# eladhoffer/convNet.pytorch

Measured on NVIDIA H100. Metric: ResNet-50 images/sec (training step, synthetic 224x224), higher is better.
Workload: dtype bf16

## Files before the change

### convnet/pytorch_b200/csrc/conv3x3.cu

```cuda
#include "common.cuh"
#include "host.h"
#include <stdlib.h>

namespace b200 {

constexpr int kHThreads = 384;
constexpr int kHTileM = 128;
constexpr int kHMaxA = 6, kHMaxB = 8;
constexpr int kHMaxTaps = 16;
constexpr int kHStatReplicas = 16;

struct HaloParams {
  int N, H, W, C, Kout;
  int RT, Wp;
  int tiles_per_img, m_tiles, n_tiles, block_n, c_chunks;
  int sa, sb;
  uint32_t a_bytes, a_box_bytes, b_bytes;
  int act;
  int has_res;
  double* stats;
  const float* bias;
  int ntaps, pad;
  int row_bytes;
  int b_stationary;
  int diag;
  uint16_t a_off[kHMaxTaps];
  uint16_t b_tap[kHMaxTaps];
};

template <int NTAPS, int KSTEPS, int BN>
__global__ void __launch_bounds__(kHThreads, 1)
conv_halo_kernel(const __grid_constant__ CUtensorMap tmX, const __grid_constant__ CUtensorMap tmB,
                 const __grid_constant__ CUtensorMap tmC, const __grid_constant__ CUtensorMap tmR,
                 const __grid_constant__ HaloParams p) {
  extern __shared__ uint8_t smem_raw[];
  __shared__ __align__(8) uint64_t a_full[kHMaxA], a_empty[kHMaxA], b_full[kHMaxB], b_empty[kHMaxB];
  __shared__ __align__(8) uint64_t res_bar, bstat_bar;

  const int warp = threadIdx.x >> 5, lane = threadIdx.x & 31;
  const uint32_t raw_addr = smem_u32(smem_raw);
  uint8_t* smem = smem_raw + (((raw_addr + 1023u) & ~1023u) - raw_addr);
  uint8_t* sA = smem;
  uint8_t* sB = sA + p.sa * p.a_bytes;
  const int b_slots = p.b_stationary ? p.c_chunks * p.ntaps : p.sb;
  uint8_t* epi = sB + b_slots * p.b_bytes;

  if (threadIdx.x == 0) {
    for (int i = 0; i < p.sa; ++i) { mbar_init(&a_full[i], 1); mbar_init(&a_empty[i], 8); }
    for (int i = 0; i < kHMaxB; ++i) { mbar_init(&b_full[i], 1); mbar_init(&b_empty[i], 8); }
    mbar_init(&bstat_bar, 1);
    mbar_init(&res_bar, 1);
    fence_mbar_init();
    prefetch_tmap(&tmX); prefetch_tmap(&tmB); prefetch_tmap(&tmC);
    if (p.has_res) prefetch_tmap(&tmR);
  }
  __syncthreads();
  pdl_wait();
  const int t_start = p.diag ? static_cast<int>(blockIdx.x) / p.n_tiles : static_cast<int>(blockIdx.x);
  const int t_step = p.diag ? static_cast<int>(gridDim.x) / p.n_tiles : static_cast<int>(gridDim.x);
  const int total_tiles = p.diag ? p.m_tiles : p.m_tiles * p.n_tiles;
  const int own_n = static_cast<int>(blockIdx.x) % p.n_tiles;

  if (warp >= 8) {
    producer_setmaxnreg();
    if (warp == 8 && lane == 0) {
      int ia = 0, ib = 0; uint32_t pa = 0, pb = 0;
      const int cw = p.row_bytes >> 1;
      if (p.b_stationary && t_start < total_tiles) {
        mbar_arrive_expect_tx(&bstat_bar, static_cast<uint32_t>(p.c_chunks * NTAPS) * p.b_bytes);
        for (int cc = 0; cc < p.c_chunks; ++cc)
          for (int t = 0; t < NTAPS; ++t)
            tma_load_3d(&tmB, &bstat_bar, sB + (cc * NTAPS + t) * p.b_bytes, cc * cw, p.b_tap[t],
                        p.diag ? own_n * p.block_n : 0);
      }
      for (int tile = t_start; tile < total_tiles; tile += t_step) {
        const int m_tile = p.diag ? tile : tile / p.n_tiles, n_tile = p.diag ? own_n : tile - m_tile * p.n_tiles;
        const int img = m_tile / p.tiles_per_img;
        const int h0 = (m_tile - img * p.tiles_per_img) * p.RT;
        for (int cc = 0; cc < p.c_chunks; ++cc) {
          mbar_wait(&a_empty[ia], pa ^ 1u);
          mbar_arrive_expect_tx(&a_full[ia], p.a_box_bytes);
          tma_load_4d(&tmX, &a_full[ia], sA + ia * p.a_bytes, (p.diag ? n_tile : cc) * cw, -p.pad, h0 - p.pad, img);
          if (++ia == p.sa) { ia = 0; pa ^= 1u; }
          if (p.b_stationary) continue;
          for (int t = 0; t < NTAPS; ++t) {
            mbar_wait(&b_empty[ib], pb ^ 1u);
            mbar_arrive_expect_tx(&b_full[ib], p.b_bytes);
            tma_load_3d(&tmB, &b_full[ib], sB + ib * p.b_bytes, cc * cw, p.b_tap[t], n_tile * p.block_n);
            if (++ib == p.sb) { ib = 0; pb ^= 1u; }
          }
        }
      }
    }
    return;
  }
  consumer_setmaxnreg();

  const int wg = warp >> 2;
  const int r_lo = wg * 64 + (warp & 3) * 16 + (lane >> 2);
  const int c_lo = 2 * (lane & 3);
  const bool leader = threadIdx.x == 0;
  const uint64_t proto = make_smem_desc(0, 16, 8u * p.row_bytes, layout_type_for_row_bytes(p.row_bytes));
  const uint32_t a_wg = (64u * wg * p.row_bytes) >> 4;
  const int nbox = BN >> 6;
  const uint32_t box_bytes = static_cast<uint32_t>(p.RT * p.W) * 128u;
  const uint32_t box_pitch = (box_bytes + 1023u) & ~1023u;
  int srow[2];
  bool in_tile[2];
#pragma unroll
  for (int h = 0; h < 2; ++h) {
    const int v = r_lo + 8 * h;
    const int ry = v / p.Wp, cx = v - ry * p.Wp;
    srow[h] = ry * p.W + cx;
    in_tile[h] = (ry < p.RT) && (cx < p.W);
  }
  const int st_col = threadIdx.x % BN;
  const int st_rows = kHTileM / (256 / BN);
  const int st_row0 = (threadIdx.x / BN) * st_rows;
  int st_ntile = -1;
  float st_s1 = 0.f, st_s2 = 0.f;
  if (p.b_stationary && t_start < total_tiles) mbar_wait(&bstat_bar, 0);

  float acc[BN / 2];
  int ia = 0, ib = 0; uint32_t pa = 0, pb = 0;
  int local = 0;
  for (int tile = t_start; tile < total_tiles; tile += t_step, ++local) {
    const int m_tile = p.diag ? tile : tile / p.n_tiles, n_tile = p.diag ? own_n : tile - m_tile * p.n_tiles;
    const int img = m_tile / p.tiles_per_img;
    const int h0 = (m_tile - img * p.tiles_per_img) * p.RT;
    const int nbase = n_tile * BN;
    if (leader && local > 0) bulk_wait_group_read0();
    named_bar_sync(1, 256);
    if (leader && p.has_res) {
      fence_proxy_async();
      mbar_arrive_expect_tx(&res_bar, static_cast<uint32_t>(nbox) * box_bytes);
      for (int b = 0; b < nbox; ++b) tma_load_4d(&tmR, &res_bar, epi + b * box_pitch, nbase + b * 64, 0, h0, img);
    }

    wgmma_fence_acc(acc);
    int rel_a = -1, rel_b = -1;
    for (int cc = 0; cc < p.c_chunks; ++cc) {
      mbar_wait(&a_full[ia], pa);
      const uint64_t da0 = proto + (smem_u32(sA + ia * p.a_bytes) >> 4) + a_wg;
#pragma unroll
      for (int t = 0; t < NTAPS; ++t) {
        uint64_t db0;
        if (p.b_stationary) {
          db0 = proto + (smem_u32(sB + (cc * NTAPS + t) * p.b_bytes) >> 4);
        } else {
          mbar_wait(&b_full[ib], pb);
          db0 = proto + (smem_u32(sB + ib * p.b_bytes) >> 4);
        }
        const uint32_t tap_inc = (static_cast<uint32_t>(p.a_off[t]) * p.row_bytes) >> 4;
        wgmma_fence();
#pragma unroll
        for (int k = 0; k < KSTEPS; ++k)
          wgmma_bf16<0, 0>(acc, da0 + tap_inc + 2 * k, db0 + 2 * k, (cc | t | k) != 0 ? 1u : 0u);
        if (!p.b_stationary || t == NTAPS - 1) {
          wgmma_commit();
          wgmma_wait<1>();
          if (rel_b >= 0) release_stage(&b_empty[rel_b], lane);
          if (rel_a >= 0) release_stage(&a_empty[rel_a], lane);
          rel_a = (t == NTAPS - 1) ? ia : -1;
          rel_b = p.b_stationary ? -1 : ib;
        }
        if (!p.b_stationary && ++ib == p.sb) { ib = 0; pb ^= 1u; }
      }
      if (++ia == p.sa) { ia = 0; pa ^= 1u; }
    }
    wgmma_wait<0>();
    wgmma_fence_acc(acc);
    if (rel_b >= 0) release_stage(&b_empty[rel_b], lane);
    if (rel_a >= 0) release_stage(&a_empty[rel_a], lane);

    if (p.has_res) mbar_wait(&res_bar, static_cast<uint32_t>(local & 1));
#pragma unroll
    for (int h = 0; h < 2; ++h) {
      if (!in_tile[h] || h0 + (r_lo + 8 * h) / p.Wp >= p.H) continue;
      const int row = srow[h];
#pragma unroll
      for (int j = 0; j < BN / 2; j += 4) {
        const int c = 2 * j + c_lo;
        {
          uint32_t* dst = reinterpret_cast<uint32_t*>(epi + (c >> 6) * box_pitch + row * 128 +
                                                      ((((c & 63) >> 3) ^ (row & 7)) << 4) + (c & 7) * 2);
          float v0 = acc[j + 2 * h], v1 = acc[j + 2 * h + 1];
          if (p.bias != nullptr) { v0 += __ldg(p.bias + nbase + c); v1 += __ldg(p.bias + nbase + c + 1); }
          if (p.has_res) {
            const float2 t2 = unpack_bf16x2(*dst);
            v0 += t2.x;
            v1 += t2.y;
          }
          *dst = pack_bf16x2(apply_act(v0, p.act), apply_act(v1, p.act));
        }
      }
    }
    fence_proxy_async();
    named_bar_sync(1, 256);
    if (leader) {
      for (int b = 0; b < nbox; ++b) tma_store_4d(&tmC, epi + b * box_pitch, nbase + b * 64, 0, h0, img);
      bulk_commit_group();
    }
    if (p.stats != nullptr) {
      if (st_ntile != n_tile) {
        if (st_ntile >= 0) {
          double* dst = p.stats + (blockIdx.x % kHStatReplicas) * 2 * p.Kout + st_ntile * BN + st_col;
          atomicAdd(dst, (double)st_s1);
          atomicAdd(dst + p.Kout, (double)st_s2);
        }
        st_ntile = n_tile; st_s1 = 0.f; st_s2 = 0.f;
      }
      const int vrows = min(p.RT, p.H - h0) * p.W;
      const uint8_t* col = epi + (st_col >> 6) * box_pitch + (st_col & 7) * 2;
      const int j = (st_col & 63) >> 3;
      const int r_end = min(st_row0 + st_rows, vrows);
      for (int r = st_row0; r < r_end; ++r) {
        const float x = __bfloat162float(*reinterpret_cast<const __nv_bfloat16*>(col + r * 128 + ((j ^ (r & 7)) << 4)));
        st_s1 += x;
        st_s2 = fmaf(x, x, st_s2);
      }
    }
  }
  if (p.stats != nullptr && st_ntile >= 0) {
    double* dst = p.stats + (blockIdx.x % kHStatReplicas) * 2 * p.Kout + st_ntile * BN + st_col;
    atomicAdd(dst, (double)st_s1);
    atomicAdd(dst + p.Kout, (double)st_s2);
  }
  if (leader) bulk_wait_group0();
}

typedef void (*HaloKernelFn)(const __grid_constant__ CUtensorMap, const __grid_constant__ CUtensorMap,
                             const __grid_constant__ CUtensorMap, const __grid_constant__ CUtensorMap,
                             const __grid_constant__ HaloParams);
static HaloKernelFn halo_kernel_for(int ntaps, int block_n) {
  if (ntaps == 9)
    return block_n == 64 ? conv_halo_kernel<9, 4, 64> : block_n == 128 ? conv_halo_kernel<9, 4, 128>
         : block_n == 256 ? conv_halo_kernel<9, 4, 256> : nullptr;
  if (ntaps == 16)
    return block_n == 64 ? conv_halo_kernel<16, 1, 64> : block_n == 128 ? conv_halo_kernel<16, 1, 128>
         : block_n == 256 ? conv_halo_kernel<16, 1, 256> : nullptr;
  return nullptr;
}

static int enc4(CUtensorMap* tm, const void* base, int C, int W, int H, int N, int b0, int b1, int b2) {
  EncodeTiledFn fn = encode_tiled_fn();
  B200_REQUIRE(fn != nullptr, B200_ERR_CUDA, "cuTensorMapEncodeTiled entry point unavailable");
  cuuint64_t dims[4] = {(cuuint64_t)C, (cuuint64_t)W, (cuuint64_t)H, (cuuint64_t)N};
  cuuint64_t strides[3] = {(cuuint64_t)C * 2, (cuuint64_t)W * C * 2, (cuuint64_t)H * W * C * 2};
  cuuint32_t box[4] = {(cuuint32_t)b0, (cuuint32_t)b1, (cuuint32_t)b2, 1};
  cuuint32_t es[4] = {1, 1, 1, 1};
  CUresult r = fn(tm, CU_TENSOR_MAP_DATA_TYPE_BFLOAT16, 4, const_cast<void*>(base), dims, strides, box, es,
                  CU_TENSOR_MAP_INTERLEAVE_NONE, swizzle_for_row_bytes(b0 * 2), CU_TENSOR_MAP_L2_PROMOTION_L2_128B,
                  CU_TENSOR_MAP_FLOAT_OOB_FILL_NONE);
  B200_REQUIRE(r == CUDA_SUCCESS, B200_ERR_CUDA, "cuTensorMapEncodeTiled(4d) failed (%d) dims=(%d,%d,%d,%d) box=(%d,%d,%d)",
               (int)r, C, W, H, N, b0, b1, b2);
  return B200_OK;
}

static bool halo_enabled() {
  static const bool enabled = !(getenv("B200_HALO") && atoi(getenv("B200_HALO")) == 0);
  return enabled;
}

bool halo_geometry_ok(int H, int W, int Cs, int R, int S, int pad) {
  if (!halo_enabled()) return false;
  const bool k3 = (R == 3 && S == 3 && pad == 1 && Cs % 64 == 0);
  const bool k4 = (R == 4 && S == 4 && pad == 0 && Cs == 16);
  if (!k3 && !k4) return false;
  const int Wp = W + S - 1;
  if (Wp > 128 || W < 8) return false;
  int RT = 128 / Wp;
  if (RT > H) RT = H;
  const int tiles = (H + RT - 1) / RT;
  return (double)H * W / (128.0 * tiles) >= 0.6;
}

bool halo_eligible(int H, int W, int Cs, int Nout, int R, int S, int pad) {
  if (!halo_geometry_ok(H, W, Cs, R, S, pad) || Nout % 64 != 0) return false;
  const int n_tiles = (Nout + 255) / 256;
  const int block_n = Nout / n_tiles;
  return Nout % n_tiles == 0 && block_n % 64 == 0 && 256 % block_n == 0;
}

int launch_halo(const void* src, const void* wmat, void* out, const void* res, const float* bias, int N, int H, int W,
                int Cs, int Nout, int R, int S, int pad, int dir, int act, double* stats, cudaStream_t stream, int window) {
  HaloParams p;
  memset(&p, 0, sizeof(p));
  p.diag = window > 0 ? 1 : 0;
  if (p.diag)
    B200_REQUIRE(window == 64 && Cs == Nout && Cs % 64 == 0 && R == 3 && S == 3, B200_ERR_UNSUPPORTED,
                 "conv halo: window mode needs window == 64, C == K, C %% 64 == 0 and a 3x3 filter (C=%d K=%d)", Cs, Nout);
  p.N = N; p.H = H; p.W = W; p.C = Cs; p.Kout = Nout;
  p.ntaps = R * S; p.pad = pad;
  p.row_bytes = (Cs == 16) ? 32 : 128;
  const int cw = p.row_bytes / 2;
  p.Wp = W + S - 1;
  p.RT = 128 / p.Wp;
  if (p.RT > H) p.RT = H;
  p.tiles_per_img = (H + p.RT - 1) / p.RT;
  p.m_tiles = N * p.tiles_per_img;
  p.n_tiles = p.diag ? Nout / 64 : (Nout + 255) / 256;
  p.block_n = Nout / p.n_tiles;
  p.c_chunks = p.diag ? 1 : Cs / cw;
  p.a_box_bytes = (uint32_t)(p.RT + R - 1) * p.Wp * p.row_bytes;
  uint32_t a_need = (uint32_t)(kHTileM + (R - 1) * p.Wp + (S - 1)) * p.row_bytes;
  if (a_need < p.a_box_bytes) a_need = p.a_box_bytes;
  p.a_bytes = (a_need + 1023u) & ~1023u;
  p.b_bytes = (uint32_t)p.block_n * p.row_bytes;
  p.act = act;
  p.has_res = res != nullptr;
  p.stats = stats;
  p.bias = bias;
  for (int r = 0; r < R; ++r)
    for (int s = 0; s < S; ++s) {
      const int t = r * S + s;
      p.b_tap[t] = (uint16_t)t;
      p.a_off[t] = (uint16_t)(dir == 0 ? r * p.Wp + s : (R - 1 - r) * p.Wp + (S - 1 - s));
    }
  const uint32_t box_pitch = (((uint32_t)(p.RT * W) * 128u) + 1023u) & ~1023u;
  const uint32_t epi_bytes = (uint32_t)(p.block_n / 64) * box_pitch;
  int budget = 212 * 1024 - (int)epi_bytes;
  const int b_all = p.c_chunks * p.ntaps * (int)p.b_bytes;
  p.b_stationary = ((p.n_tiles == 1 || p.diag) && b_all <= 80 * 1024) ? 1 : 0;
  B200_REQUIRE(!p.diag || p.b_stationary, B200_ERR_UNSUPPORTED, "conv halo: window mode expects resident weights");
  int b_region;
  if (p.b_stationary) {
    b_region = b_all;
    p.sb = 0;
    p.sa = (budget - b_region) / (int)p.a_bytes;
    if (p.sa > kHMaxA) p.sa = kHMaxA;
  } else {
    p.sa = 2;
    p.sb = (budget - p.sa * (int)p.a_bytes) / (int)p.b_bytes;
    if (p.sb > kHMaxB) p.sb = kHMaxB;
    if (p.sb >= 6 && (int)(3 * p.a_bytes + 4 * p.b_bytes) <= budget) {
      p.sa = 3;
      p.sb = (budget - 3 * (int)p.a_bytes) / (int)p.b_bytes;
      if (p.sb > kHMaxB) p.sb = kHMaxB;
    }
    b_region = p.sb * (int)p.b_bytes;
  }
  B200_REQUIRE(p.sa >= 2 && (p.b_stationary || p.sb >= 2), B200_ERR_UNSUPPORTED,
               "conv halo: shared memory budget exceeded (W=%d, block_n=%d)", W, p.block_n);
  CUtensorMap tmX, tmB, tmC, tmR;
  memset(&tmR, 0, sizeof(tmR));
  int rc = enc4(&tmX, src, Cs, W + S - 1 - 2 * pad, H + R - 1 - 2 * pad, N, cw, p.Wp, p.RT + R - 1);
  if (rc) return rc;
  {
    EncodeTiledFn fn = encode_tiled_fn();
    const int wc = p.diag ? window : Cs;
    cuuint64_t dims[3] = {(cuuint64_t)wc, (cuuint64_t)p.ntaps, (cuuint64_t)Nout};
    cuuint64_t strides[2] = {(cuuint64_t)wc * 2, (cuuint64_t)wc * p.ntaps * 2};
    cuuint32_t box[3] = {(cuuint32_t)cw, 1, (cuuint32_t)p.block_n};
    cuuint32_t es[3] = {1, 1, 1};
    CUresult r = fn(&tmB, CU_TENSOR_MAP_DATA_TYPE_BFLOAT16, 3, const_cast<void*>(wmat), dims, strides, box, es,
                    CU_TENSOR_MAP_INTERLEAVE_NONE, swizzle_for_row_bytes(p.row_bytes),
                    CU_TENSOR_MAP_L2_PROMOTION_L2_128B, CU_TENSOR_MAP_FLOAT_OOB_FILL_NONE);
    B200_REQUIRE(r == CUDA_SUCCESS, B200_ERR_CUDA, "conv halo: weight tensor map failed (%d)", (int)r);
  }
  rc = enc4(&tmC, out, Nout, W, H, N, 64, W, p.RT);
  if (rc) return rc;
  if (res) {
    rc = enc4(&tmR, res, Nout, W, H, N, 64, W, p.RT);
    if (rc) return rc;
  }
  const int smem_bytes = p.sa * (int)p.a_bytes + b_region + (int)epi_bytes + 1024;
  HaloKernelFn kfn = halo_kernel_for(p.ntaps, p.block_n);
  B200_REQUIRE(kfn != nullptr, B200_ERR_UNSUPPORTED, "conv halo: %d taps with block_n %d unsupported", p.ntaps, p.block_n);
  cudaError_t e = cudaFuncSetAttribute((const void*)kfn, cudaFuncAttributeMaxDynamicSharedMemorySize, smem_bytes);
  B200_REQUIRE(e == cudaSuccess, B200_ERR_CUDA, "conv halo: smem attribute (%d bytes): %s", smem_bytes, cudaGetErrorString(e));
  const int total = p.m_tiles * p.n_tiles;
  int grid = total < sm_count() ? total : sm_count();
  if (p.diag) {
    int per_n = sm_count() / p.n_tiles;
    if (per_n > p.m_tiles) per_n = p.m_tiles;
    if (per_n < 1) per_n = 1;
    grid = per_n * p.n_tiles;
  }
  if (getenv("B200_HALO_DEBUG"))
    fprintf(stderr, "[halo] dir=%d N=%d H=%d W=%d C=%d K=%d taps=%d block_n=%d n_tiles=%d m_tiles=%d bstat=%d diag=%d "
            "sa=%d sb=%d bias=%d res=%d act=%d stats=%d grid=%d\n", dir, N, H, W, Cs, Nout, p.ntaps, p.block_n,
            p.n_tiles, p.m_tiles, p.b_stationary, p.diag, p.sa, p.sb, bias != nullptr, res != nullptr, act,
            stats != nullptr, grid);
  b200::launch(kfn, grid, kHThreads, smem_bytes, stream, tmX, tmB, tmC, tmR, p);
  B200_CHECK_LAUNCH("conv_halo_kernel");
  return B200_OK;
}


constexpr int kWThreads = 384;
constexpr int kWMaxStages = 4;

struct HaloWgradParams {
  int N, H, W, K_out, C;
  int RT, Wp, tiles_per_img, m_tiles;
  int ntaps, pad, halo_rows;
  int x_row_bytes, cw, ncols;
  int c_chunks, k_tiles, units, splits, tiles_per_split;
  int stages;
  int window;
  uint32_t a_box_bytes, a_bytes, x_box_bytes, x_bytes;
  float* partial;
  uint16_t x_off[kHMaxTaps];
};

template <int R, int S>
__global__ void __launch_bounds__(kWThreads, 1)
conv_halo_wgrad_kernel(const __grid_constant__ CUtensorMap tmDy, const __grid_constant__ CUtensorMap tmX,
                       const __grid_constant__ HaloWgradParams p) {
  constexpr int kCols = S * 16;
  extern __shared__ uint8_t smem_raw[];
  __shared__ __align__(8) uint64_t full_bar[kWMaxStages], empty_bar[kWMaxStages];
  const int warp = threadIdx.x >> 5, lane = threadIdx.x & 31;
  const uint32_t raw_addr = smem_u32(smem_raw);
  uint8_t* smem = smem_raw + (((raw_addr + 1023u) & ~1023u) - raw_addr);
  const uint32_t stage_bytes = p.a_bytes + p.x_bytes;

  {
    uint4* z = reinterpret_cast<uint4*>(smem);
    const int n16 = static_cast<int>(p.stages * stage_bytes) >> 4;
    for (int i = threadIdx.x; i < n16; i += kWThreads) z[i] = make_uint4(0u, 0u, 0u, 0u);
  }
  if (threadIdx.x == 0) {
    for (int s = 0; s < p.stages; ++s) { mbar_init(&full_bar[s], 1); mbar_init(&empty_bar[s], 8); }
    fence_mbar_init();
    prefetch_tmap(&tmDy);
    prefetch_tmap(&tmX);
  }
  fence_proxy_async();
  __syncthreads();
  pdl_wait();

  const int split = blockIdx.x / p.units;
  const int unit = blockIdx.x - split * p.units;
  const int k_tile = unit % p.k_tiles;
  const int cc = unit / p.k_tiles;
  const int k0 = k_tile * kHTileM;
  const int t_begin = split * p.tiles_per_split;
  const int t_end = min(p.m_tiles, t_begin + p.tiles_per_split);
  const int ntiles = t_end - t_begin;
  const int nA = min(2, (p.K_out - k0 + 63) / 64);
  if (ntiles <= 0) return;

  if (warp >= 8) {
    producer_setmaxnreg();
    if (warp == 8 && lane == 0) {
      int stage = 0; uint32_t phase = 0;
      const uint32_t tx = nA * p.a_box_bytes + p.x_box_bytes;
      for (int tile = t_begin; tile < t_end; ++tile) {
        const int img = tile / p.tiles_per_img;
        const int h0 = (tile - img * p.tiles_per_img) * p.RT;
        mbar_wait(&empty_bar[stage], phase ^ 1u);
        uint8_t* sa = smem + stage * stage_bytes;
        mbar_arrive_expect_tx(&full_bar[stage], tx);
        for (int j = 0; j < nA; ++j) tma_load_4d(&tmDy, &full_bar[stage], sa + j * 16384, k0 + j * 64, 0, h0, img);
        tma_load_4d(&tmX, &full_bar[stage], sa + p.a_bytes, cc * p.cw + (p.window ? k0 : 0), -p.pad, h0 - p.pad, img);
        if (++stage == p.stages) { stage = 0; phase ^= 1u; }
      }
    }
    return;
  }
  consumer_setmaxnreg();

  const int wg = warp >> 2;
  const bool wg_on = wg < nA;
  const uint64_t protoA = make_smem_desc(0, 16384, 1024, 1);
  const uint64_t protoX = make_smem_desc(0, p.x_row_bytes, 8u * p.x_row_bytes, layout_type_for_row_bytes(p.x_row_bytes));
  uint32_t row_inc[R];
#pragma unroll
  for (int r = 0; r < R; ++r) row_inc[r] = (static_cast<uint32_t>(p.x_off[r * S]) * p.x_row_bytes) >> 4;
  const uint32_t kx_inc = (16u * p.x_row_bytes) >> 4;
  float acc[R][kCols / 2];
#pragma unroll
  for (int r = 0; r < R; ++r) wgmma_fence_acc(acc[r]);
  int stage = 0, prev = 0; uint32_t phase = 0;
  for (int i = 0; i < ntiles; ++i) {
    mbar_wait(&full_bar[stage], phase);
    if (wg_on) {
      const uint32_t a_addr = smem_u32(smem + stage * stage_bytes);
      const uint64_t da0 = protoA + ((a_addr + wg * 16384) >> 4);
      const uint64_t dx0 = protoX + ((a_addr + p.a_bytes) >> 4);
      wgmma_fence();
#pragma unroll
      for (int k = 0; k < 8; ++k) {
        const uint32_t scale = (k != 0 || i != 0) ? 1u : 0u;
#pragma unroll
        for (int r = 0; r < R; ++r)
          wgmma_bf16<1, 1>(acc[r], da0 + k * 128, dx0 + row_inc[r] + k * kx_inc, scale);
      }
      wgmma_commit();
      wgmma_wait<1>();
    }
    if (i > 0) release_stage(&empty_bar[prev], lane);
    prev = stage;
    if (++stage == p.stages) { stage = 0; phase ^= 1u; }
  }
  wgmma_wait<0>();
#pragma unroll
  for (int r = 0; r < R; ++r) wgmma_fence_acc(acc[r]);
  release_stage(&empty_bar[prev], lane);
  if (!wg_on) return;

  const int row = wg * 64 + (warp & 3) * 16 + (lane >> 2);
  const int c_lo = 2 * (lane & 3);
#pragma unroll
  for (int h = 0; h < 2; ++h) {
    float* dst = p.partial + ((static_cast<long long>(unit) * p.splits + split) * kHTileM + row + 8 * h) * p.ncols;
#pragma unroll
    for (int r = 0; r < R; ++r)
#pragma unroll
      for (int j = 0; j < kCols / 2; j += 4)
        *reinterpret_cast<float2*>(dst + r * kCols + 2 * j + c_lo) = make_float2(acc[r][j + 2 * h], acc[r][j + 2 * h + 1]);
  }
}

__global__ void __launch_bounds__(256) conv_halo_wgrad_reduce_kernel(const float* __restrict__ partial,
                                                                     float* __restrict__ dw, int K_out, int ntaps, int C,
                                                                     int cw, int k_tiles, int splits, int ncols) {
  pdl_wait();
  __shared__ float4 red[8][32];
  const int c4n = C >> 2;
  const long long total = static_cast<long long>(K_out) * ntaps * c4n;
  const int lane = threadIdx.x & 31, w = threadIdx.x >> 5, nw = blockDim.x >> 5;
  for (long long base = static_cast<long long>(blockIdx.x) * 32; base < total; base += static_cast<long long>(gridDim.x) * 32) {
    const long long idx = base + lane;
    float4 acc = make_float4(0.f, 0.f, 0.f, 0.f);
    int c = 0, tap = 0, k = 0;
    if (idx < total) {
      c = static_cast<int>(idx % c4n) * 4;
      tap = static_cast<int>((idx / c4n) % ntaps);
      k = static_cast<int>(idx / (static_cast<long long>(c4n) * ntaps));
      const int k_tile = k >> 7, row = k & 127;
      const int cc = c / cw;
      const int unit = cc * k_tiles + k_tile;
      const float* src = partial + ((static_cast<long long>(unit) * splits) * kHTileM + row) * ncols + tap * cw + (c - cc * cw);
      for (int s2 = w; s2 < splits; s2 += nw) {
        const float4 v = __ldcg(reinterpret_cast<const float4*>(src + static_cast<long long>(s2) * kHTileM * ncols));
        acc.x += v.x; acc.y += v.y; acc.z += v.z; acc.w += v.w;
      }
    }
    red[w][lane] = acc;
    __syncthreads();
    if (w == 0 && idx < total) {
      for (int j = 1; j < nw; ++j) {
        const float4 v = red[j][lane];
        acc.x += v.x; acc.y += v.y; acc.z += v.z; acc.w += v.w;
      }
      float4* d = reinterpret_cast<float4*>(dw + (static_cast<long long>(k) * ntaps + tap) * C + c);
      float4 o = *d;
      o.x += acc.x; o.y += acc.y; o.z += acc.z; o.w += acc.w;
      *d = o;
    }
    __syncthreads();
  }
}

bool halo_wgrad_eligible(int H, int W, int C, int K_out, int R, int S, int pad) {
  static const bool enabled = !(getenv("B200_HALO_WGRAD") && atoi(getenv("B200_HALO_WGRAD")) == 0);
  if (!enabled || !halo_geometry_ok(H, W, C, R, S, pad)) return false;
  return K_out % 64 == 0;
}

int launch_halo_wgrad(const void* x, const void* dy, float* dw, void* workspace, size_t workspace_bytes, int N, int H,
                      int W, int C, int K_out, int R, int S, int pad, cudaStream_t stream, int window) {
  HaloWgradParams p;
  memset(&p, 0, sizeof(p));
  p.window = window;
  if (window)
    B200_REQUIRE(window == 128 && C == K_out && C % 128 == 0, B200_ERR_UNSUPPORTED,
                 "conv halo wgrad: window mode needs window == 128 and C == K, C %% 128 == 0 (C=%d K=%d)", C, K_out);
  p.N = N; p.H = H; p.W = W; p.K_out = K_out; p.C = C;
  p.ntaps = R * S; p.pad = pad;
  p.cw = 16;
  p.x_row_bytes = p.cw * 2;
  p.ncols = p.ntaps * p.cw;
  p.Wp = W + S - 1;
  p.RT = 128 / p.Wp;
  if (p.RT > H) p.RT = H;
  p.halo_rows = p.RT + R - 1;
  p.tiles_per_img = (H + p.RT - 1) / p.RT;
  p.m_tiles = N * p.tiles_per_img;
  p.c_chunks = (window ? window : C) / p.cw;
  p.k_tiles = (K_out + kHTileM - 1) / kHTileM;
  p.units = p.c_chunks * p.k_tiles;
  int splits = sm_count() / p.units;
  if (splits < 1) splits = 1;
  if (splits > p.m_tiles) splits = p.m_tiles;
  p.tiles_per_split = (p.m_tiles + splits - 1) / splits;
  p.splits = (p.m_tiles + p.tiles_per_split - 1) / p.tiles_per_split;
  p.a_box_bytes = (uint32_t)(p.RT * p.Wp) * 128u;
  p.a_bytes = 2 * 16384;
  p.x_box_bytes = (uint32_t)(p.halo_rows * p.Wp) * p.x_row_bytes;
  int max_off = 0;
  for (int r = 0; r < R; ++r)
    for (int s = 0; s < S; ++s) {
      p.x_off[r * S + s] = (uint16_t)(r * p.Wp + s);
      if (r * p.Wp + s > max_off) max_off = r * p.Wp + s;
    }
  uint32_t x_need = (uint32_t)(kHTileM + max_off) * p.x_row_bytes;
  if (x_need < p.x_box_bytes) x_need = p.x_box_bytes;
  p.x_bytes = (x_need + 1023u) & ~1023u;
  p.stages = (212 * 1024) / (int)(p.a_bytes + p.x_bytes);
  if (p.stages > kWMaxStages) p.stages = kWMaxStages;
  B200_REQUIRE(p.stages >= 2, B200_ERR_UNSUPPORTED, "conv halo wgrad: shared memory budget exceeded (W=%d)", W);
  const size_t need = (size_t)p.units * p.splits * kHTileM * p.ncols * sizeof(float);
  B200_REQUIRE(workspace != nullptr && workspace_bytes >= need, B200_ERR_INVALID,
               "conv halo wgrad: workspace of %zu bytes needed (%zu given)", need, workspace_bytes);
  p.partial = reinterpret_cast<float*>(workspace);
  CUtensorMap tmDy, tmX;
  int rc = enc4(&tmDy, dy, K_out, W, H, N, 64, p.Wp, p.RT);
  if (rc) return rc;
  rc = enc4(&tmX, x, C, W + S - 1 - 2 * pad, H + R - 1 - 2 * pad, N, p.cw, p.Wp, p.halo_rows);
  if (rc) return rc;
  const int smem_bytes = p.stages * (int)(p.a_bytes + p.x_bytes) + 1024;
  const void* kfn = (p.ntaps == 9) ? (const void*)conv_halo_wgrad_kernel<3, 3> : (const void*)conv_halo_wgrad_kernel<4, 4>;
  cudaError_t e = cudaFuncSetAttribute(kfn, cudaFuncAttributeMaxDynamicSharedMemorySize, smem_bytes);
  B200_REQUIRE(e == cudaSuccess, B200_ERR_CUDA, "conv halo wgrad: smem attribute (%d bytes): %s", smem_bytes,
               cudaGetErrorString(e));
  if (getenv("B200_HALO_DEBUG"))
    fprintf(stderr, "[halo_wgrad] N=%d H=%d W=%d C=%d K=%d taps=%d k_tiles=%d c_chunks=%d m_tiles=%d units=%d "
            "splits=%d tiles_per_split=%d stages=%d grid=%d\n", N, H, W, C, K_out, p.ntaps, p.k_tiles, p.c_chunks,
            p.m_tiles, p.units, p.splits, p.tiles_per_split, p.stages, p.units * p.splits);
  if (p.ntaps == 9)
    b200::launch(conv_halo_wgrad_kernel<3, 3>, p.units * p.splits, kWThreads, smem_bytes, stream, tmDy, tmX, p);
  else
    b200::launch(conv_halo_wgrad_kernel<4, 4>, p.units * p.splits, kWThreads, smem_bytes, stream, tmDy, tmX, p);
  B200_CHECK_LAUNCH("conv_halo_wgrad_kernel");
  const int Cw = window ? window : C;
  const long long total = (long long)K_out * p.ntaps * (Cw / 4);
  long long blocks64 = (total + 31) / 32;
  if (blocks64 > 16LL * sm_count()) blocks64 = 16LL * sm_count();
  const int blocks = (int)blocks64;
  b200::launch(conv_halo_wgrad_reduce_kernel, blocks, 32 * wgrad_reduce_warps(p.splits), 0, stream, p.partial, dw, K_out, p.ntaps, Cw, p.cw, p.k_tiles, p.splits,
                                                            p.ncols);
  B200_CHECK_LAUNCH("conv_halo_wgrad_reduce_kernel");
  return B200_OK;
}

}
```

Before: 5474.

## Alternate consumer warpgroups over 128-row tiles so epilogue overlaps MMA

Before, both consumer warpgroups each took 64 rows of one tile. Now each warpgroup computes a full 128-row tile (two M-halves of wgmma) on its own, and the two groups alternate tile-halves. A turn barrier hands the mainloop from one group to the other, so one group's epilogue (bias, residual, activation, TMA store, BN statistics) can overlap the other's MMAs. Wide block_n is split into 128-column passes, which reloads the A tile for each pass. The epilogue buffer doubles to one per warpgroup, which takes shared memory away from the pipeline stages. Weights can no longer stay resident when block_n is split.

```diff
diff --git a/convnet/pytorch_b200/csrc/conv3x3.cu b/convnet/pytorch_b200/csrc/conv3x3.cu
--- a/convnet/pytorch_b200/csrc/conv3x3.cu
+++ b/convnet/pytorch_b200/csrc/conv3x3.cu
@@ -28,14 +28,25 @@
   uint16_t b_tap[kHMaxTaps];
 };
 
-template <int NTAPS, int KSTEPS, int BN>
+template <int KSTEPS, int SZ>
+__device__ __forceinline__ void halo_tap_mma(float (&acc)[2][SZ], uint64_t da, uint64_t db, uint32_t a_half,
+                                             uint32_t scale0) {
+  wgmma_fence();
+#pragma unroll
+  for (int k = 0; k < KSTEPS; ++k) {
+    wgmma_bf16<0, 0>(acc[0], da + 2 * k, db + 2 * k, k != 0 ? 1u : scale0);
+    wgmma_bf16<0, 0>(acc[1], da + a_half + 2 * k, db + 2 * k, k != 0 ? 1u : scale0);
+  }
+}
+
+template <int NTAPS, int KSTEPS, int WN>
 __global__ void __launch_bounds__(kHThreads, 1)
 conv_halo_kernel(const __grid_constant__ CUtensorMap tmX, const __grid_constant__ CUtensorMap tmB,
                  const __grid_constant__ CUtensorMap tmC, const __grid_constant__ CUtensorMap tmR,
                  const __grid_constant__ HaloParams p) {
   extern __shared__ uint8_t smem_raw[];
   __shared__ __align__(8) uint64_t a_full[kHMaxA], a_empty[kHMaxA], b_full[kHMaxB], b_empty[kHMaxB];
-  __shared__ __align__(8) uint64_t res_bar, bstat_bar;
+  __shared__ __align__(8) uint64_t turn_bar[2], res_bar[2], bstat_bar;
 
   const int warp = threadIdx.x >> 5, lane = threadIdx.x & 31;
   const uint32_t raw_addr = smem_u32(smem_raw);
@@ -44,12 +55,16 @@
   uint8_t* sB = sA + p.sa * p.a_bytes;
   const int b_slots = p.b_stationary ? p.c_chunks * p.ntaps : p.sb;
   uint8_t* epi = sB + b_slots * p.b_bytes;
+  const int halves = p.block_n / WN;
 
   if (threadIdx.x == 0) {
-    for (int i = 0; i < p.sa; ++i) { mbar_init(&a_full[i], 1); mbar_init(&a_empty[i], 8); }
-    for (int i = 0; i < kHMaxB; ++i) { mbar_init(&b_full[i], 1); mbar_init(&b_empty[i], 8); }
+    for (int i = 0; i < p.sa; ++i) { mbar_init(&a_full[i], 1); mbar_init(&a_empty[i], 4); }
+    for (int i = 0; i < kHMaxB; ++i) { mbar_init(&b_full[i], 1); mbar_init(&b_empty[i], 4); }
     mbar_init(&bstat_bar, 1);
-    mbar_init(&res_bar, 1);
+    for (int i = 0; i < 2; ++i) {
+      mbar_init(&res_bar[i], 1);
+      mbar_init(&turn_bar[i], 4);
+    }
     fence_mbar_init();
     prefetch_tmap(&tmX); prefetch_tmap(&tmB); prefetch_tmap(&tmC);
     if (p.has_res) prefetch_tmap(&tmR);
@@ -77,168 +92,193 @@
         const int m_tile = p.diag ? tile : tile / p.n_tiles, n_tile = p.diag ? own_n : tile - m_tile * p.n_tiles;
         const int img = m_tile / p.tiles_per_img;
         const int h0 = (m_tile - img * p.tiles_per_img) * p.RT;
+        for (int half = 0; half < halves; ++half)
+          for (int cc = 0; cc < p.c_chunks; ++cc) {
+            mbar_wait(&a_empty[ia], pa ^ 1u);
+            mbar_arrive_expect_tx(&a_full[ia], p.a_box_bytes);
+            tma_load_4d(&tmX, &a_full[ia], sA + ia * p.a_bytes, (p.diag ? n_tile : cc) * cw, -p.pad, h0 - p.pad, img);
+            if (++ia == p.sa) { ia = 0; pa ^= 1u; }
+            if (p.b_stationary) continue;
+            for (int t = 0; t < NTAPS; ++t) {
+              mbar_wait(&b_empty[ib], pb ^ 1u);
+              mbar_arrive_expect_tx(&b_full[ib], p.b_bytes);
+              tma_load_3d(&tmB, &b_full[ib], sB + ib * p.b_bytes, cc * cw, p.b_tap[t], n_tile * p.block_n + half * WN);
+              if (++ib == p.sb) { ib = 0; pb ^= 1u; }
+            }
+          }
+      }
+    }
+    return;
+  }
+  consumer_setmaxnreg();
+
+  const int wg = warp >> 2;
+  const int wt = threadIdx.x & 127;
+  const int r_lo = (warp & 3) * 16 + (lane >> 2);
+  const int c_lo = 2 * (lane & 3);
+  const bool leader = wt == 0;
+  const uint64_t proto = make_smem_desc(0, 16, 8u * p.row_bytes, layout_type_for_row_bytes(p.row_bytes));
+  const uint32_t a_half = (64u * p.row_bytes) >> 4;
+  constexpr int nbox = WN / 64;
+  const uint32_t box_bytes = static_cast<uint32_t>(p.RT * p.W) * 128u;
+  const uint32_t box_pitch = (box_bytes + 1023u) & ~1023u;
+  uint8_t* epi_w = epi + wg * nbox * box_pitch;
+  const int st_col = wt % WN;
+  const int st_row0 = (wt / WN) * WN;
+  int st_nbase = -1;
+  float st_s1 = 0.f, st_s2 = 0.f;
+  auto flush_stats = [&]() {
+    double* dst = p.stats + (blockIdx.x % kHStatReplicas) * 2 * p.Kout + st_nbase + st_col;
+    atomicAdd(dst, (double)st_s1);
+    atomicAdd(dst + p.Kout, (double)st_s2);
+    st_s1 = 0.f; st_s2 = 0.f;
+  };
+  if (p.b_stationary && t_start < total_tiles) mbar_wait(&bstat_bar, 0);
+
+  float acc[2][WN / 2];
+  int local = 0;
+  for (int tile = t_start; tile < total_tiles; tile += t_step) {
+    for (int half = 0; half < halves; ++half, ++local) {
+      if ((local & 1) != wg) continue;
+      const int m_tile = p.diag ? tile : tile / p.n_tiles, n_tile = p.diag ? own_n : tile - m_tile * p.n_tiles;
+      const int img = m_tile / p.tiles_per_img;
+      const int h0 = (m_tile - img * p.tiles_per_img) * p.RT;
+      const int nbase = n_tile * p.block_n + half * WN;
+      const int mine = local >> 1;
+      if (leader && mine > 0) bulk_wait_group_read0();
+      named_bar_sync(1 + wg, 128);
+      if (leader && p.has_res) {
+        fence_proxy_async();
+        mbar_arrive_expect_tx(&res_bar[wg], static_cast<uint32_t>(nbox) * box_bytes);
+        for (int b = 0; b < nbox; ++b) tma_load_4d(&tmR, &res_bar[wg], epi_w + b * box_pitch, nbase + b * 64, 0, h0, img);
+      }
+
+      const int pos_a = local * p.c_chunks;
+      int ia = pos_a % p.sa;
+      uint32_t pa = static_cast<uint32_t>(pos_a / p.sa) & 1u;
+      int ib = 0;
+      uint32_t pb = 0;
+      if (!p.b_stationary) {
+        const int pos_b = pos_a * NTAPS;
+        ib = pos_b % p.sb;
+        pb = static_cast<uint32_t>(pos_b / p.sb) & 1u;
+      }
+      if (local > 0) mbar_wait(&turn_bar[wg], static_cast<uint32_t>((local - 1) >> 1) & 1u);
+
+      wgmma_fence_acc(acc[0]);
+      wgmma_fence_acc(acc[1]);
+      int rel_a = -1, rel_b = -1;
+      if (p.b_stationary) {
         for (int cc = 0; cc < p.c_chunks; ++cc) {
-          mbar_wait(&a_empty[ia], pa ^ 1u);
-          mbar_arrive_expect_tx(&a_full[ia], p.a_box_bytes);
-          tma_load_4d(&tmX, &a_full[ia], sA + ia * p.a_bytes, (p.diag ? n_tile : cc) * cw, -p.pad, h0 - p.pad, img);
+          mbar_wait(&a_full[ia], pa);
+          const uint64_t da0 = proto + (smem_u32(sA + ia * p.a_bytes) >> 4);
+          const uint64_t db0 = proto + (smem_u32(sB + cc * NTAPS * p.b_bytes) >> 4);
+#pragma unroll
+          for (int t = 0; t < NTAPS; ++t)
+            halo_tap_mma<KSTEPS>(acc, da0 + ((static_cast<uint32_t>(p.a_off[t]) * p.row_bytes) >> 4),
+                                 db0 + ((t * p.b_bytes) >> 4), a_half, (cc | t) != 0 ? 1u : 0u);
+          wgmma_commit();
+          wgmma_wait<1>();
+          if (rel_a >= 0) release_stage(&a_empty[rel_a], lane);
+          rel_a = ia;
           if (++ia == p.sa) { ia = 0; pa ^= 1u; }
-          if (p.b_stationary) continue;
+        }
+      } else {
+        for (int cc = 0; cc < p.c_chunks; ++cc) {
+          mbar_wait(&a_full[ia], pa);
+          const uint64_t da0 = proto + (smem_u32(sA + ia * p.a_bytes) >> 4);
+#pragma unroll
           for (int t = 0; t < NTAPS; ++t) {
-            mbar_wait(&b_empty[ib], pb ^ 1u);
-            mbar_arrive_expect_tx(&b_full[ib], p.b_bytes);
-            tma_load_3d(&tmB, &b_full[ib], sB + ib * p.b_bytes, cc * cw, p.b_tap[t], n_tile * p.block_n);
+            mbar_wait(&b_full[ib], pb);
+            halo_tap_mma<KSTEPS>(acc, da0 + ((static_cast<uint32_t>(p.a_off[t]) * p.row_bytes) >> 4),
+                                 proto + (smem_u32(sB + ib * p.b_bytes) >> 4), a_half, (cc | t) != 0 ? 1u : 0u);
+            wgmma_commit();
+            wgmma_wait<1>();
+            if (rel_b >= 0) release_stage(&b_empty[rel_b], lane);
+            if (rel_a >= 0) release_stage(&a_empty[rel_a], lane);
+            rel_a = (t == NTAPS - 1) ? ia : -1;
+            rel_b = ib;
             if (++ib == p.sb) { ib = 0; pb ^= 1u; }
           }
+          if (++ia == p.sa) { ia = 0; pa ^= 1u; }
         }
       }
-    }
-    return;
-  }
-  consumer_setmaxnreg();
-
-  const int wg = warp >> 2;
-  const int r_lo = wg * 64 + (warp & 3) * 16 + (lane >> 2);
-  const int c_lo = 2 * (lane & 3);
-  const bool leader = threadIdx.x == 0;
-  const uint64_t proto = make_smem_desc(0, 16, 8u * p.row_bytes, layout_type_for_row_bytes(p.row_bytes));
-  const uint32_t a_wg = (64u * wg * p.row_bytes) >> 4;
-  const int nbox = BN >> 6;
-  const uint32_t box_bytes = static_cast<uint32_t>(p.RT * p.W) * 128u;
-  const uint32_t box_pitch = (box_bytes + 1023u) & ~1023u;
-  int srow[2];
-  bool in_tile[2];
-#pragma unroll
-  for (int h = 0; h < 2; ++h) {
-    const int v = r_lo + 8 * h;
-    const int ry = v / p.Wp, cx = v - ry * p.Wp;
-    srow[h] = ry * p.W + cx;
-    in_tile[h] = (ry < p.RT) && (cx < p.W);
-  }
-  const int st_col = threadIdx.x % BN;
-  const int st_rows = kHTileM / (256 / BN);
-  const int st_row0 = (threadIdx.x / BN) * st_rows;
-  int st_ntile = -1;
-  float st_s1 = 0.f, st_s2 = 0.f;
-  if (p.b_stationary && t_start < total_tiles) mbar_wait(&bstat_bar, 0);
-
-  float acc[BN / 2];
-  int ia = 0, ib = 0; uint32_t pa = 0, pb = 0;
-  int local = 0;
-  for (int tile = t_start; tile < total_tiles; tile += t_step, ++local) {
-    const int m_tile = p.diag ? tile : tile / p.n_tiles, n_tile = p.diag ? own_n : tile - m_tile * p.n_tiles;
-    const int img = m_tile / p.tiles_per_img;
-    const int h0 = (m_tile - img * p.tiles_per_img) * p.RT;
-    const int nbase = n_tile * BN;
-    if (leader && local > 0) bulk_wait_group_read0();
-    named_bar_sync(1, 256);
-    if (leader && p.has_res) {
+      __syncwarp();
+      if (lane == 0) mbar_arrive(&turn_bar[wg ^ 1]);
+      wgmma_wait<0>();
+      wgmma_fence_acc(acc[0]);
+      wgmma_fence_acc(acc[1]);
+      if (rel_b >= 0) release_stage(&b_empty[rel_b], lane);
+      if (rel_a >= 0) release_stage(&a_empty[rel_a], lane);
+
+      const int vrows = min(p.RT, p.H - h0) * p.W;
+      int srow[2][2];
+#pragma unroll
+      for (int mh = 0; mh < 2; ++mh)
+#pragma unroll
+        for (int h = 0; h < 2; ++h) {
+          const int v = mh * 64 + r_lo + 8 * h;
+          const int ry = v / p.Wp, cx = v - ry * p.Wp;
+          srow[mh][h] = (ry < p.RT && cx < p.W) ? ry * p.W + cx : p.RT * p.W;
+        }
+      if (p.has_res) mbar_wait(&res_bar[wg], static_cast<uint32_t>(mine & 1));
+#pragma unroll
+      for (int j = 0; j < WN / 2; j += 4) {
+        const int c = 2 * j + c_lo;
+        float bias0 = 0.f, bias1 = 0.f;
+        if (p.bias != nullptr) { bias0 = __ldg(p.bias + nbase + c); bias1 = __ldg(p.bias + nbase + c + 1); }
+#pragma unroll
+        for (int mh = 0; mh < 2; ++mh)
+#pragma unroll
+          for (int h = 0; h < 2; ++h) {
+            const int row = srow[mh][h];
+            if (row >= vrows) continue;
+            uint32_t* dst = reinterpret_cast<uint32_t*>(epi_w + (c >> 6) * box_pitch + row * 128 +
+                                                        ((((c & 63) >> 3) ^ (row & 7)) << 4) + (c & 7) * 2);
+            float v0 = acc[mh][j + 2 * h] + bias0, v1 = acc[mh][j + 2 * h + 1] + bias1;
+            if (p.has_res) {
+              const float2 t2 = unpack_bf16x2(*dst);
+              v0 += t2.x;
+              v1 += t2.y;
+            }
+            *dst = pack_bf16x2(apply_act(v0, p.act), apply_act(v1, p.act));
+          }
+      }
       fence_proxy_async();
-      mbar_arrive_expect_tx(&res_bar, static_cast<uint32_t>(nbox) * box_bytes);
-      for (int b = 0; b < nbox; ++b) tma_load_4d(&tmR, &res_bar, epi + b * box_pitch, nbase + b * 64, 0, h0, img);
-    }
-
-    wgmma_fence_acc(acc);
-    int rel_a = -1, rel_b = -1;
-    for (int cc = 0; cc < p.c_chunks; ++cc) {
-      mbar_wait(&a_full[ia], pa);
-      const uint64_t da0 = proto + (smem_u32(sA + ia * p.a_bytes) >> 4) + a_wg;
-#pragma unroll
-      for (int t = 0; t < NTAPS; ++t) {
-        uint64_t db0;
-        if (p.b_stationary) {
-          db0 = proto + (smem_u32(sB + (cc * NTAPS + t) * p.b_bytes) >> 4);
-        } else {
-          mbar_wait(&b_full[ib], pb);
-          db0 = proto + (smem_u32(sB + ib * p.b_bytes) >> 4);
+      named_bar_sync(1 + wg, 128);
+      if (leader) {
+        for (int b = 0; b < nbox; ++b) tma_store_4d(&tmC, epi_w + b * box_pitch, nbase + b * 64, 0, h0, img);
+        bulk_commit_group();
+      }
+      if (p.stats != nullptr) {
+        if (st_nbase != nbase) {
+          if (st_nbase >= 0) flush_stats();
+          st_nbase = nbase;
         }
-        const uint32_t tap_inc = (static_cast<uint32_t>(p.a_off[t]) * p.row_bytes) >> 4;
-        wgmma_fence();
-#pragma unroll
-        for (int k = 0; k < KSTEPS; ++k)
-          wgmma_bf16<0, 0>(acc, da0 + tap_inc + 2 * k, db0 + 2 * k, (cc | t | k) != 0 ? 1u : 0u);
-        if (!p.b_stationary || t == NTAPS - 1) {
-          wgmma_commit();
-          wgmma_wait<1>();
-          if (rel_b >= 0) release_stage(&b_empty[rel_b], lane);
-          if (rel_a >= 0) release_stage(&a_empty[rel_a], lane);
-          rel_a = (t == NTAPS - 1) ? ia : -1;
-          rel_b = p.b_stationary ? -1 : ib;
+        const uint8_t* col = epi_w + (st_col >> 6) * box_pitch + (st_col & 7) * 2;
+        const int j = (st_col & 63) >> 3;
+        const int r_end = min(st_row0 + WN, vrows);
+#pragma unroll 8
+        for (int r = st_row0; r < r_end; ++r) {
+          const float x = __bfloat162float(*reinterpret_cast<const __nv_bfloat16*>(col + r * 128 + ((j ^ (r & 7)) << 4)));
+          st_s1 += x;
+          st_s2 = fmaf(x, x, st_s2);
         }
-        if (!p.b_stationary && ++ib == p.sb) { ib = 0; pb ^= 1u; }
-      }
-      if (++ia == p.sa) { ia = 0; pa ^= 1u; }
-    }
-    wgmma_wait<0>();
-    wgmma_fence_acc(acc);
-    if (rel_b >= 0) release_stage(&b_empty[rel_b], lane);
-    if (rel_a >= 0) release_stage(&a_empty[rel_a], lane);
-
-    if (p.has_res) mbar_wait(&res_bar, static_cast<uint32_t>(local & 1));
-#pragma unroll
-    for (int h = 0; h < 2; ++h) {
-      if (!in_tile[h] || h0 + (r_lo + 8 * h) / p.Wp >= p.H) continue;
-      const int row = srow[h];
-#pragma unroll
-      for (int j = 0; j < BN / 2; j += 4) {
-        const int c = 2 * j + c_lo;
-        {
-          uint32_t* dst = reinterpret_cast<uint32_t*>(epi + (c >> 6) * box_pitch + row * 128 +
-                                                      ((((c & 63) >> 3) ^ (row & 7)) << 4) + (c & 7) * 2);
-          float v0 = acc[j + 2 * h], v1 = acc[j + 2 * h + 1];
-          if (p.bias != nullptr) { v0 += __ldg(p.bias + nbase + c); v1 += __ldg(p.bias + nbase + c + 1); }
-          if (p.has_res) {
-            const float2 t2 = unpack_bf16x2(*dst);
-            v0 += t2.x;
-            v1 += t2.y;
-          }
-          *dst = pack_bf16x2(apply_act(v0, p.act), apply_act(v1, p.act));
-        }
-      }
-    }
-    fence_proxy_async();
-    named_bar_sync(1, 256);
-    if (leader) {
-      for (int b = 0; b < nbox; ++b) tma_store_4d(&tmC, epi + b * box_pitch, nbase + b * 64, 0, h0, img);
-      bulk_commit_group();
-    }
-    if (p.stats != nullptr) {
-      if (st_ntile != n_tile) {
-        if (st_ntile >= 0) {
-          double* dst = p.stats + (blockIdx.x % kHStatReplicas) * 2 * p.Kout + st_ntile * BN + st_col;
-          atomicAdd(dst, (double)st_s1);
-          atomicAdd(dst + p.Kout, (double)st_s2);
-        }
-        st_ntile = n_tile; st_s1 = 0.f; st_s2 = 0.f;
-      }
-      const int vrows = min(p.RT, p.H - h0) * p.W;
-      const uint8_t* col = epi + (st_col >> 6) * box_pitch + (st_col & 7) * 2;
-      const int j = (st_col & 63) >> 3;
-      const int r_end = min(st_row0 + st_rows, vrows);
-      for (int r = st_row0; r < r_end; ++r) {
-        const float x = __bfloat162float(*reinterpret_cast<const __nv_bfloat16*>(col + r * 128 + ((j ^ (r & 7)) << 4)));
-        st_s1 += x;
-        st_s2 = fmaf(x, x, st_s2);
-      }
-    }
-  }
-  if (p.stats != nullptr && st_ntile >= 0) {
-    double* dst = p.stats + (blockIdx.x % kHStatReplicas) * 2 * p.Kout + st_ntile * BN + st_col;
-    atomicAdd(dst, (double)st_s1);
-    atomicAdd(dst + p.Kout, (double)st_s2);
-  }
+      }
+    }
+  }
+  if (p.stats != nullptr && st_nbase >= 0) flush_stats();
   if (leader) bulk_wait_group0();
 }
 
 typedef void (*HaloKernelFn)(const __grid_constant__ CUtensorMap, const __grid_constant__ CUtensorMap,
                              const __grid_constant__ CUtensorMap, const __grid_constant__ CUtensorMap,
                              const __grid_constant__ HaloParams);
-static HaloKernelFn halo_kernel_for(int ntaps, int block_n) {
+static HaloKernelFn halo_kernel_for(int ntaps, int wn) {
   if (ntaps == 9)
-    return block_n == 64 ? conv_halo_kernel<9, 4, 64> : block_n == 128 ? conv_halo_kernel<9, 4, 128>
-         : block_n == 256 ? conv_halo_kernel<9, 4, 256> : nullptr;
+    return wn == 64 ? conv_halo_kernel<9, 4, 64> : wn == 128 ? conv_halo_kernel<9, 4, 128> : nullptr;
   if (ntaps == 16)
-    return block_n == 64 ? conv_halo_kernel<16, 1, 64> : block_n == 128 ? conv_halo_kernel<16, 1, 128>
-         : block_n == 256 ? conv_halo_kernel<16, 1, 256> : nullptr;
+    return wn == 64 ? conv_halo_kernel<16, 1, 64> : wn == 128 ? conv_halo_kernel<16, 1, 128> : nullptr;
   return nullptr;
 }
 
@@ -306,7 +346,8 @@
   uint32_t a_need = (uint32_t)(kHTileM + (R - 1) * p.Wp + (S - 1)) * p.row_bytes;
   if (a_need < p.a_box_bytes) a_need = p.a_box_bytes;
   p.a_bytes = (a_need + 1023u) & ~1023u;
-  p.b_bytes = (uint32_t)p.block_n * p.row_bytes;
+  const int wn = p.block_n < 128 ? p.block_n : 128;
+  p.b_bytes = (uint32_t)wn * p.row_bytes;
   p.act = act;
   p.has_res = res != nullptr;
   p.stats = stats;
@@ -318,10 +359,10 @@
       p.a_off[t] = (uint16_t)(dir == 0 ? r * p.Wp + s : (R - 1 - r) * p.Wp + (S - 1 - s));
     }
   const uint32_t box_pitch = (((uint32_t)(p.RT * W) * 128u) + 1023u) & ~1023u;
-  const uint32_t epi_bytes = (uint32_t)(p.block_n / 64) * box_pitch;
+  const uint32_t epi_bytes = 2u * (uint32_t)(wn / 64) * box_pitch;
   int budget = 212 * 1024 - (int)epi_bytes;
   const int b_all = p.c_chunks * p.ntaps * (int)p.b_bytes;
-  p.b_stationary = ((p.n_tiles == 1 || p.diag) && b_all <= 80 * 1024) ? 1 : 0;
+  p.b_stationary = ((p.n_tiles == 1 || p.diag) && wn == p.block_n && b_all <= 80 * 1024) ? 1 : 0;
   B200_REQUIRE(!p.diag || p.b_stationary, B200_ERR_UNSUPPORTED, "conv halo: window mode expects resident weights");
   int b_region;
   if (p.b_stationary) {
@@ -351,7 +392,7 @@
     const int wc = p.diag ? window : Cs;
     cuuint64_t dims[3] = {(cuuint64_t)wc, (cuuint64_t)p.ntaps, (cuuint64_t)Nout};
     cuuint64_t strides[2] = {(cuuint64_t)wc * 2, (cuuint64_t)wc * p.ntaps * 2};
-    cuuint32_t box[3] = {(cuuint32_t)cw, 1, (cuuint32_t)p.block_n};
+    cuuint32_t box[3] = {(cuuint32_t)cw, 1, (cuuint32_t)wn};
     cuuint32_t es[3] = {1, 1, 1};
     CUresult r = fn(&tmB, CU_TENSOR_MAP_DATA_TYPE_BFLOAT16, 3, const_cast<void*>(wmat), dims, strides, box, es,
                     CU_TENSOR_MAP_INTERLEAVE_NONE, swizzle_for_row_bytes(p.row_bytes),
@@ -365,7 +406,7 @@
     if (rc) return rc;
   }
   const int smem_bytes = p.sa * (int)p.a_bytes + b_region + (int)epi_bytes + 1024;
-  HaloKernelFn kfn = halo_kernel_for(p.ntaps, p.block_n);
+  HaloKernelFn kfn = halo_kernel_for(p.ntaps, wn);
   B200_REQUIRE(kfn != nullptr, B200_ERR_UNSUPPORTED, "conv halo: %d taps with block_n %d unsupported", p.ntaps, p.block_n);
   cudaError_t e = cudaFuncSetAttribute((const void*)kfn, cudaFuncAttributeMaxDynamicSharedMemorySize, smem_bytes);
   B200_REQUIRE(e == cudaSuccess, B200_ERR_CUDA, "conv halo: smem attribute (%d bytes): %s", smem_bytes, cudaGetErrorString(e));
```

After: 5556, median of 6. 1.01x the previous value.
